# cvg/EMAP

Measured on AMD Instinct MI355X. Metric: ray-samples/sec (UDF MLP + composite), higher is better.
Workload: dtype f16x3 (split-fp16 MFMA, 3 passes, fp32 accumulate)

## Files before the change

### emap_amd/csrc/emap_common.h

```cpp
#pragma once
#include <hip/hip_runtime.h>
#include <stdint.h>
#include <stdio.h>
#include "../../include/emap_hip.h"


namespace emap {
constexpr float F16X3_WS = 8192.0f;
constexpr float F16_LO_SCALE = 2048.0f;

void set_error(const char* fmt, ...);
int check_launch(const char* what);

inline bool attr_needed(uint64_t& mask) {
    int d = 0;
    if (hipGetDevice(&d) != hipSuccess || d < 0 || d > 63) return true;
    if (mask & (1ull << d)) return false;
    mask |= 1ull << d;
    return true;
}
inline int raise_lds_limit(uint64_t& mask, const void* fn, int bytes = 160 * 1024) {
    if (attr_needed(mask) && hipFuncSetAttribute(fn, hipFuncAttributeMaxDynamicSharedMemorySize, bytes) != hipSuccess) {
        set_error("hipFuncSetAttribute(MaxDynamicSharedMemorySize) failed");
        return EMAP_E_LAUNCH;
// ... 63 lines not shown
    const float* rays_d;
    const float* z;
    int32_t n_per_ray;
    int32_t mid;
    const float* sample_dist;
    const float* near;
    const float* far;
    const float* t_rand;
    int32_t coarse;
    int32_t zero_n;
    int32_t* zero_cnt;
};

struct CompositeArgs {
    const float *rays_o, *rays_d, *z, *udf, *grad, *depth_scale, *sample_dist;
    int N, S;
    float inv_s, beta, gamma, car;
    int anneal;
    float flip_sat, near_surface, sparse_scale, background;
    int has_bg;
    const float *var_p, *beta_p, *gamma_p;
    float beta_min;
    EmapCompositeOut out;
    float* partials;
    const float* sched;
};

struct CompositeFuse {
    CompositeArgs c;
    int32_t* ray_cnt;
    int32_t* done_cnt;
};
constexpr int REV_MAX_WG = 768;
constexpr int REV_WG_CAP_4W = REV_MAX_WG * 2 / 3;
constexpr int COMP_LIST_MAX = 8192;
constexpr int COMP_FUSED_MAX_S = 256;
inline long long comp_list_entries(long long P, int S) {
    const long long tiles = (P + 63) / 64, grid = tiles < REV_WG_CAP_4W ? tiles : REV_WG_CAP_4W;
    return ((tiles + grid - 1) / (grid > 0 ? grid : 1)) * (64 / (S > 0 ? S : 1) + 2);
}
struct StepArgs {
    const float *rays_o, *rays_d;
    const float *z, *udf;
    const float *z_prev, *udf_prev;
    float *z_merged, *udf_merged;
    const float *near, *far, *t_rand;
    float* sample_dist;
    float* z_new;
    float* z_final;
    int N, n, m;
    float inv_s, beta, gamma;
    int32_t* err;
};
int launch_sampler_step(bool coarse, bool tail, const StepArgs& a, hipStream_t st, bool plain = false);

struct IsLaunch {
    const float *rays_o, *rays_d, *near, *far, *t_rand;
    float* sample_dist;
    const float* udf_coarse;
    float* z_final;
    int32_t N, Sc, m, steps;
};
constexpr int IS_NOT_FUSED = 1;
int launch_importance(const NetLayout& L, const void* packed, int prec, const IsLaunch& q, hipStream_t st, int32_t* err_flags);
int set_fused_sampling(int on);
int fused_sampling_mode();
int launch_mlp(const NetLayout& L, const void* packed, int prec, const PointSource& src, int64_t P,
               float* udf, float* grad3, hipStream_t st, int32_t* err_flags = nullptr, void* scratch = nullptr,
               const CompositeFuse* fuse = nullptr);
int launch_null_direction(const float* g, int64_t n, int k, float* dir, hipStream_t st);
int launch_lattice_points(int N, int64_t first, int64_t count, float* xyz, hipStream_t st);
size_t compact_workspace_bytes(int64_t n);
int launch_compact_append(const float* df, const float* xyz, int64_t n, int64_t first_index, float thr, int inclusive, float* out_xyz,
                          float* out_df, int64_t* out_idx, int64_t capacity, int64_t* state, void* workspace, hipStream_t st);
int launch_jitter_points(const float* x, const float* noise, int64_t n, int k, float delta, float* out, hipStream_t st);
int launch_shift_points(const float* x, const float* df, const float* normal, int64_t n, float* out, hipStream_t st);

constexpr int VJP_PT = 32;
#ifndef EMAP_VJP_CHUNK_TILES
#define EMAP_VJP_CHUNK_TILES 16384
#endif
constexpr int VJP_CHUNK_TILES = EMAP_VJP_CHUNK_TILES;
constexpr __host__ __device__ int vjp_slab_planes(bool split_f16, bool sweep_mx) { return split_f16 && !sweep_mx ? 6 : 4; }
__device__ __forceinline__ float vjp_scale_from(const uint32_t* absmax) {
    const float mu = __builtin_bit_cast(float, absmax[0]), mg = __builtin_bit_cast(float, absmax[1]);
    const float m = fmaxf(mg, mu * (1.0f / 64.0f));
    if (!(m > 1e-30f) || !(m < 1e30f)) return 1.0f;
    int e;
    (void)frexpf(m, &e);
    return ldexpf(1.0f, -e);
}
constexpr int WGRAD_MAX_JOBS = 2 * EMAP_MAX_LIN;
struct VjpLayout {
    int32_t a_rt[EMAP_MAX_LIN + 1], a_off[EMAP_MAX_LIN + 1];
    int32_t z_rt[EMAP_MAX_LIN], z_off[EMAP_MAX_LIN];
    int32_t s_off[EMAP_MAX_LIN];
    int32_t a_tile_kb, z_tile_kb, s_slab_kb;
    long long lo_a_delta, lo_z_delta;
};
void build_vjp_layout(const NetLayout& L, VjpLayout* V);
struct WgradJob {
    int32_t layer, part;
    int32_t z_off, z_rt;
    int32_t a_off, a_ct;
    int32_t first_wg, n_slices;
    int32_t part_off;
    int32_t bias_off;
};
struct WgradPlan {
    WgradJob jobs[WGRAD_MAX_JOBS];
    int n_jobs, total_wg;
    int job_h[EMAP_MAX_LIN], job_pe[EMAP_MAX_LIN];
    size_t partial_floats;
};
struct VjpSweep {
    PointSource src;
    int64_t P;
    int tile0, n_tiles;
    const float *d_udf, *d_grad;
    const VjpLayout* V;
    char *stash_a, *stash_z, *stash_s;
    int grid;
    const uint32_t* absmax;
    float* ldot;
};

bool mlp_uses_rev(const NetLayout& L, int prec, int64_t P);
int set_grad_mode(int mode);
extern int g_prof_clk_device;
long long* prof_clk_here();
extern long long* g_prof_clk;
constexpr int REV_SG_BYTES_PER_NC = 3072;
inline size_t rev_scratch_bytes(const NetLayout& L) {
    return L.has_rev ? (size_t)REV_WG_CAP_4W * ((size_t)(L.n_lin - 1) * (size_t)(L.H / 32) * (2 * REV_SG_BYTES_PER_NC) + 8192) : 0;
}

int launch_sample_pdf(const float* bins, const float* weights, int N, int n, int m, float* samples, int64_t* inds, int32_t* err,
                      hipStream_t st, const float* u = nullptr);
int launch_upsample(const float* rays_o, const float* rays_d, const float* z, const float* udf, int N, int n, int m, const float* sample_dist,
                    float inv_s, float beta, float gamma, float* z_new, int64_t* inds, int32_t* err, hipStream_t st);
int launch_upsample_plain(const float* z, const float* udf, int N, int n, int m, const float* sample_dist, float beta, float gamma, float* z_new,
                          int64_t* inds, int32_t* err, hipStream_t st);
int launch_merge(const float* z, const float* z_new, const float* udf, const float* udf_new, int N, int n, int m, float* z_out, float* udf_out,
                 int64_t* perm, hipStream_t st);
int launch_coarse(const float* near, const float* far, const float* t_rand, int N, int n_samples, float* z, float* sample_dist, hipStream_t st);
int fill_composite_args(const float* rays_o, const float* rays_d, const float* z, const float* udf, const float* grad3, const float* depth_scale,
                        int N, int S, const float* sample_dist, const EmapRenderParams& p, const EmapCompositeOut* out, float* partials,
                        CompositeArgs* a, const float* sched = nullptr);
int launch_composite(const float* rays_o, const float* rays_d, const float* z, const float* udf, const float* grad3, const float* depth_scale,
                     int N, int S, const float* sample_dist, const EmapRenderParams& p, const EmapCompositeOut* out, float* partials,
                     int32_t* err, hipStream_t st, const float* sched = nullptr);
int launch_composite_reduce(const CompositeArgs& a, int32_t* err, hipStream_t st);
int launch_composite_bwd(const float* rays_o, const float* rays_d, const float* z, const float* udf, const float* grad3, const float* depth_scale,
                         int N, int S, const float* sample_dist, const EmapRenderParams* p, const EmapCompositeGrads* gr, float* d_udf,
                         float* d_grad3, float* partials, uint32_t* absmax, hipStream_t st, const float* sched = nullptr);
int launch_embed(const float* x, int64_t P, int L, float* pe, hipStream_t st);
void linspace_host(float start, float end, int steps, float* out);
int launch_sample_rays(const EmapRayDataset* ds, int img_idx, int batch, int importance, uint64_t seed, uint64_t offset, uint64_t* counter,
                       const int64_t* pixels_in, const EmapRayBatch* out, hipStream_t st);
int check_train_images(const int32_t* images, int n_train, int n_images);
int launch_sample_rays_train(const EmapRayDataset* ds, const int32_t* train_images, int n_train, int32_t* perm, int64_t* epoch_tag, int batch,
                             int importance, uint64_t seed, uint64_t* counter, const int64_t* pixels_in, const EmapRayBatch* out, hipStream_t st);
int gen_rays_count(const EmapRayDataset* ds, int resolution_level, int64_t* n, int* h, int* w);
int launch_gen_rays_at(const EmapRayDataset* ds, int img_idx, int resolution_level, int64_t first, int64_t count, float* rays_o, float* rays_d,
                       float* depth_scale, hipStream_t st);
int launch_train_stats(const float* edge, const float* true_edge, const float* scalars, int N, float d_scale, float* d_edge, float* stats,
// ... 32 lines not shown
```

### emap_amd/csrc/udf_mlp_vjp.inc

```
#pragma once

__device__ __forceinline__ void asm_gload4(uint32_t& dst, int voff, const char* sbase) {
    asm volatile("s_nop 4\n\tglobal_load_dword %0, %1, %2" : "=v"(dst) : "v"(voff), "s"(sbase) : "memory");
}
template <int N>
__device__ __forceinline__ void asm_wait_unit(u32x4& a, u32x4& b, u32x4& c, u32x4& d, u32x2& e, u32x2& f, u32x2& g, u32x2& h, uint32_t& i) {
    asm volatile("s_waitcnt vmcnt(%c9)" : "+v"(a), "+v"(b), "+v"(c), "+v"(d), "+v"(e), "+v"(f), "+v"(g), "+v"(h), "+v"(i) : "i"(N) : "memory");
}


struct VjpArgs {
    MlpArgs m;
    const float* d_udf;
    const float* d_grad;
    char* stash_a;
    char* stash_z;
    char* stash_s;
    const uint32_t* absmax;
    float* ldot;
    VjpLayout V;
    int32_t tile0;
    const char* swm;
    int32_t swm_unit[EMAP_MAX_LIN], swm_t_unit[EMAP_MAX_LIN];
};

template <int H, int MODE, int NW, bool SMX_ = false>
__global__ __launch_bounds__(NW * 64, NW == 8 ? 1 : 2) void udf_mlp_vjp_kernel(const VjpArgs va) {
    using T = typename Prec<MODE>::T;
    using V8 = typename Prec<MODE>::V;
    const MlpArgs& a = va.m;
    constexpr int NPART = Prec<MODE>::NPART;
    constexpr bool SCALED = (NPART == 2);
    constexpr float LO_SCALE = (MODE == EMAP_PREC_F16X3) ? F16_LO_SCALE : 1.0f;
    constexpr int NCT = 4;
    constexpr int NKS = H / 32;
    constexpr int NPAIR = H / 32;
    constexpr int NFR = 2 * NPART;
    constexpr int PD = 2;
    constexpr int PPW = NPAIR / NW;
    constexpr int KQ = NKS / NW;
    static_assert(PPW == 1 && PPW * NW == NPAIR && KQ * NW == NKS && NW >= 4, "waves per workgroup");
    constexpr bool SMX = SMX_ && MODE == EMAP_PREC_F16X3 && H == 256;
    constexpr int NSLAB = vjp_slab_planes(MODE == EMAP_PREC_F16X3, SMX);
    constexpr bool SLABLO = NSLAB > 4;
    typedef uint32_t u32x8 __attribute__((ext_vector_type(8)));

    extern __shared__ __attribute__((aligned(16))) char smem[];
    constexpr int XB = NKS * NCT * NPART * FRAG_BYTES;
    constexpr int PB = PE_KS * NCT * NPART * FRAG_BYTES;
    constexpr bool PP = (NW == 8);
    char* const xb0 = smem;
    char* const xb1 = smem + (PP ? XB : 0);
    char* pebuf = smem + (PP ? 2 : 1) * XB;
    float* red = reinterpret_cast<float*>(PP ? smem + 2 * XB + PB : smem);
    int cur = 0;

    const int tid = threadIdx.x;
    const int lane = tid & 63;
    const int wave = __builtin_amdgcn_readfirstlane(tid >> 6);
    const int g = lane >> 4;
    const int j = lane & 15;
    const int wvoff = lane * 16;
    const char* wbase = uniform_ptr(a.frags);
    const char* tbase = uniform_ptr(a.tfrags);
    const int n_hidden = a.n_lin - 1;
    const char* xr = xb0 + lane * 16;
    const int xm_lane = g * (NCT * NPART * FRAG_BYTES) + FRAG_BYTES;
    const char* xmr = xb0 + xm_lane;
    const char* per = pebuf + lane * 16;
    const int p0 = wave * PPW;
    V8 sel[2];
#pragma unroll
    for (int h = 0; h < 2; ++h)
#pragma unroll
        for (int e = 0; e < 8; ++e) sel[h][e] = ((j >> 2) == g && e == 4 * h + (j & 3)) ? (T)1.0f : (T)0.0f;
    char* const slab = va.stash_s + (size_t)blockIdx.x * ((size_t)va.V.s_slab_kb * 1024);
    const float Kscale = vjp_scale_from(va.absmax);

    clock_stamp(a.clk, 2);
    V8 hd[PD][NFR];
    auto load_head = [&](const char* wb) __attribute__((always_inline)) {
#pragma unroll
        for (int sp = 0; sp < PD; ++sp)
#pragma unroll
            for (int f = 0; f < NFR; ++f) {
                typedef const V8 __attribute__((address_space(1))) * gptr_t;
                hd[sp][f] = *(gptr_t)(uintptr_t)(wb + (sp * NFR + f) * FRAG_BYTES + wvoff);
            }
    };
    u32x2 hd6r[4];
    uint32_t hasc = 0;
    auto load_head_mx = [&](const char* wbh, const char* wm) __attribute__((always_inline)) {
        typedef const V8 __attribute__((address_space(1))) * gptr_t;
        typedef const u32x2 __attribute__((address_space(1))) * g2_t;
        typedef const uint32_t __attribute__((address_space(1))) * g1_t;
#pragma unroll
        for (int sp = 0; sp < PD; ++sp)
#pragma unroll
            for (int t = 0; t < 2; ++t) hd[sp][t] = *(gptr_t)(uintptr_t)(wbh + (sp * NFR + 2 * t) * FRAG_BYTES + wvoff);
#pragma unroll
        for (int t = 0; t < 2; ++t)
#pragma unroll
            for (int pt = 0; pt < 2; ++pt) {
                hd[t][2 + pt] = *(gptr_t)(uintptr_t)(wm + (2 * t + pt) * 1024 + wvoff);
                hd6r[2 * t + pt] = *(g2_t)(uintptr_t)(wm + 4096 + (2 * t + pt) * 512 + lane * 8);
            }
        hasc = *(g1_t)(uintptr_t)(wm + 6144 + lane * 4);
    };
    auto head_after_fwd = [&](int l) __attribute__((always_inline)) {
        int ln = l + 1;
        while (ln < n_hidden && p0 >= a.layer[ln].n_pairs) ++ln;
        const LayerDesc Ln = a.layer[ln < n_hidden ? ln : a.n_lin - 1];
        if constexpr (SMX) {
            if (ln >= n_hidden) return;
            if (!Ln.pe_ks) {
                load_head_mx(wbase + (size_t)(Ln.frag_off + p0 * Ln.h_ks * NFR) * FRAG_BYTES,
                             va.swm + (size_t)(va.swm_unit[ln] + p0 * (NKS / 4)) * SWM_UNIT_BYTES);
                return;
            }
        }
        const int first = (ln < n_hidden) ? p0 * (Ln.pe_ks + Ln.h_ks) : Ln.pe_ks + KQ * wave;
        load_head(wbase + (size_t)(Ln.frag_off + first * NFR) * FRAG_BYTES);
    };
    auto head_after_bwd = [&](int b, int tile) __attribute__((always_inline)) {
        int bn = b - 1;
        while (bn >= 1 && p0 >= a.layer[bn - 1].n_pairs) --bn;
        if (bn >= 1) {
            if constexpr (SMX) load_head_mx(tbase + (size_t)(a.t_off[bn] + p0 * NKS * NFR) * FRAG_BYTES,
                                            va.swm + (size_t)(va.swm_t_unit[bn] + p0 * (NKS / 4)) * SWM_UNIT_BYTES);
            else load_head(tbase + (size_t)(a.t_off[bn] + p0 * NKS * NFR) * FRAG_BYTES);
        }
        else if (tile + (int)gridDim.x < a.n_tiles) head_after_fwd(-1);
    };
    if ((int)blockIdx.x < a.n_tiles) head_after_fwd(-1);
    for (int i = tid * 16; i < (PP ? 2 : 1) * XB; i += NW * 64 * 16) *reinterpret_cast<f32x4*>(smem + i) = f32x4{0.f, 0.f, 0.f, 0.f};
    __syncthreads();
    for (int tile = blockIdx.x; tile < a.n_tiles; tile += gridDim.x) {
        const long long pbase = ((long long)va.tile0 + tile) * VJP_PT;
        char* const sa = va.stash_a + (size_t)tile * ((size_t)va.V.a_tile_kb * 1024);
        char* const sz = va.stash_z + (size_t)tile * ((size_t)va.V.z_tile_kb * 1024);
        constexpr bool LO_STASH = (NPART == 2) && !SMX;
        const bool stash_lo = LO_STASH && va.V.lo_a_delta != 0;
        auto stash_store = [&](char* level_pair, const V8 (&x)[4], int n_rt) __attribute__((always_inline)) {
            const f32x4 z4 = {0.f, 0.f, 0.f, 0.f};
#pragma unroll
            for (int h = 0; h < 2; ++h) {
                if (h < n_rt) {
                    f32x4 d[4];
#pragma unroll
                    for (int ct = 0; ct < 4; ++ct) d[ct] = mfma16(x[ct], sel[h], z4);
#pragma unroll
                    for (int ks = 0; ks < 2; ++ks) {
                        V8 v;
#pragma unroll
                        for (int e = 0; e < 8; ++e) v[e] = (T)d[2 * ks + (e >> 2)][e & 3];
                        *reinterpret_cast<V8*>(level_pair + (h * 2 + ks) * 1024 + lane * 16) = v;
                    }
                }
            }
        };

        if (wave < NCT) {
            const int ct = wave;
            int gq = g;
            asm volatile("" : "+v"(gq));
            float xs[3], vd[3] = {0.f, 0.f, 0.f};
            long long pp = pbase + 16 * (ct & 1) + j;
            const bool valid = pp < a.P;
            if (!valid) pp = a.P - 1;
            load_point(a.src, pp, a.scale, xs);
            if (ct >= 2 && valid) {
                vd[0] = va.d_grad[3 * pp + 0] * Kscale;
                vd[1] = va.d_grad[3 * pp + 1] * Kscale;
                vd[2] = va.d_grad[3 * pp + 2] * Kscale;
            }
            V8 f[PE_KS][NPART];
#pragma unroll
            for (int q = 0; q < 8; ++q) {
                const PeAngle ang = pe_angle(xs, 8 * gq + q, a.multires);
                float v0, v1;
                if (ct < 2) {
                    pe_pair(ang, xs, a.multires, 0, v0, v1);
                } else {
                    const float vc = (ang.c == 0) ? vd[0] : ((ang.c == 1) ? vd[1] : vd[2]);
                    const bool r0 = ang.a == 3 * a.multires, r1 = ang.a == 3 * a.multires + 1;
                    v0 = ang.is_ang ? ang.f * ang.cs * vc : (r0 ? vd[0] : (r1 ? vd[2] : 0.0f));
                    v1 = ang.is_ang ? -ang.f * ang.sn * vc : (r0 ? vd[1] : 0.0f);
                }
                const T h0 = (T)v0, h1 = (T)v1;
                f[q >> 2][0][2 * (q & 3)] = h0;
                f[q >> 2][0][2 * (q & 3) + 1] = h1;
                if constexpr (NPART == 2) {
                    f[q >> 2][1][2 * (q & 3)] = (T)((v0 - (float)h0) * LO_SCALE);
                    f[q >> 2][1][2 * (q & 3) + 1] = (T)((v1 - (float)h1) * LO_SCALE);
                }
            }
#pragma unroll
            for (int sp = 0; sp < PE_KS; ++sp)
#pragma unroll
                for (int pt = 0; pt < NPART; ++pt)
                    *reinterpret_cast<V8*>(pebuf + ((sp * NCT + ct) * NPART + pt) * FRAG_BYTES + lane * 16) = f[sp][pt];
        }
        __syncthreads();
        if (wave >= NW - PE_KS) {
            const int sp = wave - (NW - PE_KS);
            V8 c4[NCT];
#pragma unroll
            for (int ct = 0; ct < NCT; ++ct) c4[ct] = *reinterpret_cast<const V8*>(per + ((sp * NCT + ct) * NPART + 0) * FRAG_BYTES);
            stash_store(sa + (size_t)va.V.a_off[0] * 1024 + (2 * sp) * 2048, c4, 2);
            if constexpr (LO_STASH) {
                if (stash_lo) {
#pragma unroll
                    for (int ct = 0; ct < NCT; ++ct) c4[ct] = *reinterpret_cast<const V8*>(per + ((sp * NCT + ct) * NPART + (NPART - 1)) * FRAG_BYTES);
                    stash_store(sa + va.V.lo_a_delta + (size_t)va.V.a_off[0] * 1024 + (2 * sp) * 2048, c4, 2);
                }
            }
        }

        f32x4 acc[2][NCT];
        f32x4 accx[SCALED ? 2 : 1][NCT];
        V8 o[NCT][NPART];
        const f32x4 zero4 = {0.f, 0.f, 0.f, 0.f};

        auto zval = [&](int t, int ct, int r) __attribute__((always_inline)) -> float {
            if constexpr (SCALED) return fmaf(accx[t][ct][r], 1.0f / LO_SCALE, acc[t][ct][r]);
            else return acc[t][ct][r];
        };

        auto k_run_p = [&](auto ns_c, auto npe_c, auto init_c, auto pre_c, const char* wb, int xs0, int pes0, const float* bp) __attribute__((always_inline)) {
            constexpr int NS = decltype(ns_c)::value;
            constexpr int NPE = decltype(npe_c)::value;
            constexpr bool INIT = decltype(init_c)::value;
            constexpr bool PRE = decltype(pre_c)::value;
            V8 af[PD + 1][NFR];
            auto load_a = [&](auto s_c) __attribute__((always_inline)) {
                constexpr int s = decltype(s_c)::value;
#pragma unroll
                for (int f = 0; f < NFR; ++f) asm_gload16(af[s % (PD + 1)][f], wvoff, wb + (s * NFR + f) * FRAG_BYTES);
            };
            if constexpr (PRE) {
#pragma unroll
                for (int sp = 0; sp < PD; ++sp)
#pragma unroll
                    for (int f = 0; f < NFR; ++f) af[sp][f] = hd[sp][f];
            } else static_for<PD>([&](auto i_c) __attribute__((always_inline)) { if constexpr (decltype(i_c)::value < NS) load_a(i_c); });
            f32x4 i0 = zero4, i1 = zero4;
            if constexpr (INIT) {
                i0 = *reinterpret_cast<const f32x4*>(bp);
                i1 = *reinterpret_cast<const f32x4*>(bp + 16);
            }
            const char* xq = xr + xs0 * (NCT * NPART * FRAG_BYTES);
            const char* pq = per + pes0 * (NCT * NPART * FRAG_BYTES);
            V8 bh[NCT], bl[NCT];
            static_for<NS>([&](auto s_c) __attribute__((always_inline)) {
                constexpr int s = decltype(s_c)::value;
                constexpr int sa_ = s % (PD + 1);
                if constexpr (s == 0 && INIT) asm volatile("" : "+v"(i0), "+v"(i1));
                if constexpr (s + PD < NS) load_a(std::integral_constant<int, s + PD>{});
                constexpr bool is_pe = s < NPE;
                constexpr int sb = is_pe ? s : s - NPE;
#pragma unroll
                for (int ct = 0; ct < NCT; ++ct) {
                    const char* base = is_pe ? pq : xq;
                    bh[ct] = *reinterpret_cast<const V8*>(base + ((sb * NCT + ct) * NPART + 0) * FRAG_BYTES);
                    bl[ct] = *reinterpret_cast<const V8*>(base + ((sb * NCT + ct) * NPART + (NPART - 1)) * FRAG_BYTES);
                }
                {
                    constexpr int younger = ((s + PD < NS) ? PD : (NS - 1 - s)) * NFR;
#pragma unroll
                    for (int f = 0; f < NFR; f += 2) asm_wait_vm<younger>(af[sa_][f], af[sa_][f + 1]);
                }
                if constexpr (s == 0) {
#pragma unroll
                    for (int c2 = 0; c2 < NCT; ++c2) {
                        acc[0][c2] = (c2 < 2) ? i0 : zero4;
                        acc[1][c2] = (c2 < 2) ? i1 : zero4;
                        if constexpr (SCALED) { accx[0][c2] = zero4; accx[1][c2] = zero4; }
                    }
                }
                if constexpr (NPART == 1) {
#pragma unroll
                    for (int ct = 0; ct < NCT; ++ct) {
                        acc[0][ct] = mfma16(af[sa_][0], bh[ct], acc[0][ct]);
                        acc[1][ct] = mfma16(af[sa_][1], bh[ct], acc[1][ct]);
                    }
                } else {
#pragma unroll
                    for (int ct = 0; ct < NCT; ++ct) {
                        if constexpr (SCALED) { accx[0][ct] = mfma16(af[sa_][0], bl[ct], accx[0][ct]); accx[1][ct] = mfma16(af[sa_][2], bl[ct], accx[1][ct]); }
                        else { acc[0][ct] = mfma16(af[sa_][0], bl[ct], acc[0][ct]); acc[1][ct] = mfma16(af[sa_][2], bl[ct], acc[1][ct]); }
                    }
#pragma unroll
                    for (int ct = 0; ct < NCT; ++ct) {
                        acc[0][ct] = mfma16(af[sa_][0], bh[ct], acc[0][ct]);
                        acc[1][ct] = mfma16(af[sa_][2], bh[ct], acc[1][ct]);
                    }
#pragma unroll
// ... 149 lines not shown
                            const auto s02 = __builtin_amdgcn_permlane32_swap(x0, x2, false, false);
                            const auto s13 = __builtin_amdgcn_permlane32_swap(x1, x3, false, false);
                            const auto w01 = __builtin_amdgcn_permlane16_swap(s02[0], s13[0], false, false);
                            const auto w23 = __builtin_amdgcn_permlane16_swap(s02[1], s13[1], false, false);
                            blk[pt][0 * 4 + d] = w01[0]; blk[pt][1 * 4 + d] = w01[1]; blk[pt][2 * 4 + d] = w23[0]; blk[pt][3 * 4 + d] = w23[1];
                        }
                    auto block_max = [&](const u32x16& v) __attribute__((always_inline)) -> float {
                        uint32_t mb = 0;
#pragma unroll
                        for (int q = 0; q < 16; ++q)
                            asm("v_pk_maximum3_f16 %0, %1, %2, %2 neg_lo:[0,0,1] neg_hi:[0,0,1]" : "=v"(mb) : "v"(mb), "v"(v[q]));
                        const h2 m = __builtin_bit_cast(h2, mb);
                        return fmaxf((float)m[0], (float)m[1]);
                    };
                    const uint32_t sbh = mx6_scale_bits(block_max(blk[0])), sbl = mx6_scale_bits(block_max(blk[1]));
                    const u32x6 qh = __builtin_amdgcn_cvt_scalef32_pk32_fp6_f16(__builtin_bit_cast(f16x32, blk[0]), __builtin_bit_cast(float, sbh));
                    const u32x6 ql = __builtin_amdgcn_cvt_scalef32_pk32_fp6_f16(__builtin_bit_cast(f16x32, blk[1]), __builtin_bit_cast(float, sbl));
                    char* const dst = xbuf + ((p0 * NCT + g) * NPART + 1) * FRAG_BYTES;
                    *reinterpret_cast<u32x4*>(dst + j * 16) = u32x4{qh[0], qh[1], qh[2], qh[3]};
                    *reinterpret_cast<u32x4*>(dst + 256 + j * 16) = u32x4{ql[0], ql[1], ql[2], ql[3]};
                    *reinterpret_cast<u32x2*>(dst + 512 + j * 8) = u32x2{qh[4], qh[5]};
                    *reinterpret_cast<u32x2*>(dst + 640 + j * 8) = u32x2{ql[4], ql[5]};
                    *reinterpret_cast<uint32_t*>(dst + 768 + j * 4) = (sbh >> 23) | ((((sbl >> 23) - 11u) & 0xffu) << 8);
                }
            }
            __syncthreads();
            if constexpr (PP) { cur ^= 1; xr = (cur ? xb1 : xb0) + lane * 16; xmr = (cur ? xb1 : xb0) + xm_lane; }
        };
        using yes_t = std::true_type;
        using no_t = std::false_type;
        u32x4 sgv[4];
        auto load_slab = [&](const char* src) __attribute__((always_inline)) {
            const char* sb = uniform_ptr(src);
            static_for<4>([&](auto c_c) __attribute__((always_inline)) {
                constexpr int c = decltype(c_c)::value;
                asm_gload16_sc1<c * 1024>(sgv[c], wvoff, sb);
            });
        };
        auto wait_slab = [&]() __attribute__((always_inline)) {
            asm volatile("s_waitcnt vmcnt(0)" : "+v"(sgv[0]), "+v"(sgv[1]), "+v"(sgv[2]), "+v"(sgv[3]) : : "memory");
        };

        for (int l = 0; l < n_hidden; ++l) {
            const LayerDesc L = a.layer[l];
            const int kind = (L.h_ks == 0) ? KIND_FIRST : (L.pe_ks ? KIND_SKIP : KIND_NORMAL);
            const int p = p0;
            if (p < L.n_pairs) {
                const float* bp = a.bias + l * H + 32 * p + 4 * g;
                const int ns = L.pe_ks + L.h_ks;
                const char* wb = wbase + (size_t)(L.frag_off + p * ns * NFR) * FRAG_BYTES;
                if constexpr (SMX) {
                    const char* wm = va.swm + (size_t)(va.swm_unit[l] + p * (NKS / 4)) * SWM_UNIT_BYTES;
                    if (kind == KIND_NORMAL) k_run_mx(std::integral_constant<int, 1>{}, std::integral_constant<int, NKS / 4>{}, yes_t{}, 0, wb, wm, bp);
                    else if (kind == KIND_SKIP) {
                        k_run_p(std::integral_constant<int, PE_KS>{}, std::integral_constant<int, PE_KS>{}, yes_t{}, yes_t{}, wb, 0, 0, bp);
                        k_run_mx(std::integral_constant<int, 2>{}, std::integral_constant<int, NKS / 4>{}, no_t{}, 0, wb + (size_t)PE_KS * NFR * FRAG_BYTES, wm, bp);
                    } else k_run_p(std::integral_constant<int, PE_KS>{}, std::integral_constant<int, PE_KS>{}, yes_t{}, yes_t{}, wb, 0, 0, bp);
                } else {
                if (kind == KIND_NORMAL) k_run_p(std::integral_constant<int, NKS>{}, std::integral_constant<int, 0>{}, yes_t{}, yes_t{}, wb, 0, 0, bp);
                else if (kind == KIND_SKIP) k_run_p(std::integral_constant<int, PE_KS + NKS>{}, std::integral_constant<int, PE_KS>{}, yes_t{}, yes_t{}, wb, 0, 0, bp);
                else k_run_p(std::integral_constant<int, PE_KS>{}, std::integral_constant<int, PE_KS>{}, yes_t{}, yes_t{}, wb, 0, 0, bp);
                }
                head_after_fwd(l);
                uint32_t bk[SLABLO ? 24 : 16];
                static_for<8>([&](auto q_c) __attribute__((always_inline)) {
                    constexpr int q = decltype(q_c)::value, t = q >> 2, r = q & 3;
                    float a0, s0, a1, s1;
                    softplus_sig_fast(zval(t, 0, r), a0, s0);
                    softplus_sig_fast(zval(t, 1, r), a1, s1);
                    const float t0 = s0 * zval(t, 2, r), t1 = s1 * zval(t, 3, r);
                    put1(0, 4 * t + r, a0);
                    put1(1, 4 * t + r, a1);
                    typedef T T2 __attribute__((ext_vector_type(2)));
                    const T2 ap2 = {put1(2, 4 * t + r, t0), put1(3, 4 * t + r, t1)};
                    bk[2 * q] = __builtin_bit_cast(uint32_t, ap2);
                    bk[2 * q + 1] = __builtin_bit_cast(uint32_t, __builtin_amdgcn_cvt_pknorm_u16(s0, s1));
                    if constexpr (SLABLO) {
                        const T2 lo2 = {(T)((t0 - (float)ap2[0]) * LO_SCALE), (T)((t1 - (float)ap2[1]) * LO_SCALE)};
                        bk[16 + q] = __builtin_bit_cast(uint32_t, lo2);
                    }
                });
                {
                    const V8 xh[4] = {o[0][0], o[1][0], o[2][0], o[3][0]};
                    stash_store(sa + (size_t)va.V.a_off[l + 1] * 1024 + (2 * p) * 2048, xh, 2);
                }
                if constexpr (LO_STASH) {
                    if (stash_lo) {
                        const V8 xl[4] = {o[0][NPART - 1], o[1][NPART - 1], o[2][NPART - 1], o[3][NPART - 1]};
                        stash_store(sa + va.V.lo_a_delta + (size_t)va.V.a_off[l + 1] * 1024 + (2 * p) * 2048, xl, 2);
                    }
                }
                u32x4* dst = reinterpret_cast<u32x4*>(slab + ((size_t)(l * NPAIR + p) * NSLAB) * 1024 + lane * 16);
#pragma unroll
                for (int c = 0; c < NSLAB; ++c) dst[c * 64] = u32x4{bk[4 * c], bk[4 * c + 1], bk[4 * c + 2], bk[4 * c + 3]};
            }
            publish(L.n_pairs);
        }

        float hpart[NCT];
        {
            const LayerDesc L = a.layer[a.n_lin - 1];
            const char* wb = wbase + (size_t)(L.frag_off + (L.pe_ks + KQ * wave) * NFR) * FRAG_BYTES;
            if constexpr (SMX) {
#pragma unroll
                for (int ct = 0; ct < NCT; ++ct) hpart[ct] = 0.f;
                if (wave < NKS / 4) {
                    k_run_mx(std::integral_constant<int, 0>{}, std::integral_constant<int, 1>{}, no_t{}, wave, wbase + (size_t)L.frag_off * FRAG_BYTES,
                             va.swm + (size_t)va.swm_unit[a.n_lin - 1] * SWM_UNIT_BYTES, nullptr);
#pragma unroll
                    for (int ct = 0; ct < NCT; ++ct) hpart[ct] = zval(0, ct, 0);
                }
            } else {
            k_run_p(std::integral_constant<int, KQ>{}, std::integral_constant<int, 0>{}, no_t{}, yes_t{}, wb, KQ * wave, 0, nullptr);
#pragma unroll
            for (int ct = 0; ct < NCT; ++ct) hpart[ct] = zval(0, ct, 0);
            }
            if (L.pe_ks && wave < PE_KS) {
                const char* wp = wbase + (size_t)(L.frag_off + wave * NFR) * FRAG_BYTES;
                k_run(std::integral_constant<int, 1>{}, std::integral_constant<int, 1>{}, no_t{}, wp, 0, wave, nullptr);
#pragma unroll
                for (int ct = 0; ct < NCT; ++ct) hpart[ct] += zval(0, ct, 0);
            }
            head_after_bwd(a.n_lin - 1, tile);
            if constexpr (!PP) __syncthreads();
            if (g == 0) {
#pragma unroll
                for (int ct = 0; ct < NCT; ++ct) red[(wave * NCT + ct) * 16 + j] = hpart[ct];
            }
        }
        __syncthreads();
        float seed[NCT];
        {
            float hs[NCT];
#pragma unroll
            for (int ct = 0; ct < NCT; ++ct) {
                float v = 0.f;
#pragma unroll
                for (int w = 0; w < NW; ++w) v += red[(w * NCT + ct) * 16 + j];
                hs[ct] = v;
            }
            const float b_last = a.bias[(a.n_lin - 1) * H];
            const float inv_scale = 1.0f / a.scale;
            bool bad = false;
#pragma unroll
            for (int c = 0; c < 2; ++c) {
                const long long pp = pbase + 16 * c + j;
                const float h = hs[c] + b_last, hp = hs[c + 2];
                float u1, u2;
                if (a.udf_type == EMAP_UDF_ABS) { u1 = (h > 0.f) ? 1.f : ((h < 0.f) ? -1.f : 0.f); u2 = 0.f; }
                else if (a.udf_type == EMAP_UDF_SQUARE) { u1 = 2.f * h; u2 = 2.f; }
                else { u1 = 1.f; u2 = 0.f; }
                const bool valid = pp < a.P;
                const float du = valid ? va.d_udf[pp] * Kscale : 0.f;
                seed[c] = valid ? fmaf(du * inv_scale, u1, u2 * hp) : 0.f;
                seed[c + 2] = valid ? u1 : 0.f;
                bad |= valid && !(fabsf(h) + fabsf(hp) <= 3.0e38f);
            }
            if (wave == 0 && g == 0) flag_nonfinite(a.err, bad);
            if (wave == 0 && g == 0) {
                float d = seed[0] * hs[0] + seed[1] * hs[1] + seed[2] * hs[2] + seed[3] * hs[3];
#pragma unroll
                for (int off = 8; off > 0; off >>= 1) d += __shfl_xor(d, off);
                if (j == 0) va.ldot[va.tile0 + tile] = d;
            }
        }
        if (wave == 0) {
            V8 xs[4];
#pragma unroll
            for (int ct = 0; ct < NCT; ++ct) {
                const T hi = (T)seed[ct];
#pragma unroll
                for (int e = 0; e < 8; ++e) xs[ct][e] = (T)0.0f;
                xs[ct][0] = (g == 0) ? hi : (T)0.0f;
                xs[ct][1] = (g == 0) ? (T)(seed[ct] - (float)hi) : (T)0.0f;
            }
            stash_store(sz + (size_t)va.V.z_off[a.n_lin - 1] * 1024, xs, 1);
            if constexpr (LO_STASH) {
                if (stash_lo) {
#pragma unroll
                    for (int ct = 0; ct < NCT; ++ct)
#pragma unroll
                        for (int e = 0; e < 8; ++e) xs[ct][e] = (T)0.0f;
                    stash_store(sz + va.V.lo_z_delta + (size_t)va.V.z_off[a.n_lin - 1] * 1024, xs, 1);
                }
            }
        }

        for (int b = a.n_lin - 1; b >= 1; --b) {
            const int lz = b - 1;
            const int p = p0;
            if (p < a.layer[lz].n_pairs) {
                load_slab(slab + ((size_t)(lz * NPAIR + p) * NSLAB) * 1024);
                if (b == a.n_lin - 1) {
                    const f32x4 w0 = *reinterpret_cast<const f32x4*>(a.wlast + 32 * p + 4 * g);
                    const f32x4 w1 = *reinterpret_cast<const f32x4*>(a.wlast + 32 * p + 16 + 4 * g);
#pragma unroll
                    for (int ct = 0; ct < NCT; ++ct) {
                        acc[0][ct] = w0 * seed[ct];
                        acc[1][ct] = w1 * seed[ct];
                        if constexpr (SCALED) { accx[0][ct] = zero4; accx[1][ct] = zero4; }
                    }
                } else {
                    const char* wb = tbase + (size_t)(a.t_off[b] + p * NKS * NFR) * FRAG_BYTES;
                    if constexpr (SMX) k_run_mx(std::integral_constant<int, 0>{}, std::integral_constant<int, NKS / 4>{}, yes_t{}, 0, wb,
                                                va.swm + (size_t)(va.swm_t_unit[b] + p * (NKS / 4)) * SWM_UNIT_BYTES, nullptr);
                    else k_run_p(std::integral_constant<int, NKS>{}, std::integral_constant<int, 0>{}, no_t{}, yes_t{}, wb, 0, 0, nullptr);
                }
                wait_slab();
                u32x4 aplo[2];
                if constexpr (SLABLO) {
                    const char* lp = uniform_ptr(slab + ((size_t)(lz * NPAIR + p) * NSLAB + 4) * 1024);
                    asm_gload16_sc1<0>(aplo[0], wvoff, lp);
                    asm_gload16_sc1<1024>(aplo[1], wvoff, lp);
                    asm volatile("s_waitcnt vmcnt(0)" : "+v"(aplo[0]), "+v"(aplo[1]) : : "memory");
                }
                if (b != a.n_lin - 1) head_after_bwd(b, tile);
                static_for<8>([&](auto q_c) __attribute__((always_inline)) {
                    constexpr int q = decltype(q_c)::value, t = q >> 2, r = q & 3;
                    typedef T T2 __attribute__((ext_vector_type(2)));
                    const uint32_t apk = sgv[q >> 1][2 * (q & 1)], spk = sgv[q >> 1][2 * (q & 1) + 1];
                    const T2 ap2 = __builtin_bit_cast(T2, apk);
                    float ap0 = (float)ap2[0], ap1 = (float)ap2[1];
                    if constexpr (SLABLO) {
                        const uint32_t lok = aplo[q >> 2][q & 3];
                        const T2 lo2 = __builtin_bit_cast(T2, lok);
                        ap0 = fmaf((float)lo2[0], 1.0f / LO_SCALE, ap0);
                        ap1 = fmaf((float)lo2[1], 1.0f / LO_SCALE, ap1);
                    }
                    const float s0 = (float)(spk & 0xffffu) * (1.0f / 65535.0f);
                    const float s1 = (float)(spk >> 16) * (1.0f / 65535.0f);
                    const float av0 = zval(t, 0, r), av1 = zval(t, 1, r), at0 = zval(t, 2, r), at1 = zval(t, 3, r);
                    const float zb0 = fmaf(100.0f * (1.0f - s0) * ap0, at0, s0 * av0);
                    const float zb1 = fmaf(100.0f * (1.0f - s1) * ap1, at1, s1 * av1);
                    put1(0, 4 * t + r, zb0);
                    put1(1, 4 * t + r, zb1);
                    put1(2, 4 * t + r, s0 * at0);
                    put1(3, 4 * t + r, s1 * at1);
                });
                {
                    const V8 xh[4] = {o[0][0], o[1][0], o[2][0], o[3][0]};
                    stash_store(sz + (size_t)va.V.z_off[lz] * 1024 + (2 * p) * 2048, xh, 2);
                }
                if constexpr (LO_STASH) {
                    if (stash_lo) {
                        const V8 xl[4] = {o[0][NPART - 1], o[1][NPART - 1], o[2][NPART - 1], o[3][NPART - 1]};
                        stash_store(sz + va.V.lo_z_delta + (size_t)va.V.z_off[lz] * 1024 + (2 * p) * 2048, xl, 2);
                    }
                }
            }
            if (b > 1) publish(a.layer[lz].n_pairs);
        }
        __syncthreads();
    }
    clock_stamp(a.clk, 3);
}

template <int H, int MODE, int NW, bool SMX_ = false>
static int launch_vjp_sweep_t(const NetLayout& L, const void* packed, const VjpSweep& s, hipStream_t st, int32_t* err) {
    constexpr int NPART = Prec<MODE>::NPART;
    VjpArgs va;
    memset(&va, 0, sizeof(va));
    va.m = fill_mlp_args(L, packed, L.frag_off_bytes, L.t_frag_off_bytes, s.src, s.P, err);
    va.m.n_tiles = s.n_tiles; va.tile0 = s.tile0;
    va.m.clk = prof_clk_here();
    va.d_udf = s.d_udf; va.d_grad = s.d_grad; va.stash_a = s.stash_a; va.stash_z = s.stash_z; va.stash_s = s.stash_s; va.absmax = s.absmax; va.ldot = s.ldot; va.V = *s.V;
    va.swm = static_cast<const char*>(packed) + L.swm_off_bytes;
    for (int l = 0; l < L.n_lin; ++l) { va.swm_unit[l] = L.swm_unit[l]; va.swm_t_unit[l] = L.swm_t_unit[l]; }
    const size_t lds = (NW == 8) ? (size_t)(2 * (H / 32) + PE_KS) * 4 * NPART * FRAG_BYTES + (size_t)NW * 4 * 16 * 4
                                 : (size_t)((H / 32) + PE_KS) * 4 * NPART * FRAG_BYTES;
    auto kern = udf_mlp_vjp_kernel<H, MODE, NW, SMX_>;
    static uint64_t attr_mask = 0;
    const int rc = raise_lds_limit(attr_mask, reinterpret_cast<const void*>(kern));
    if (rc) return rc;
    if (s.n_tiles <= 0) return EMAP_OK;
    hipLaunchKernelGGL(kern, dim3(s.grid < s.n_tiles ? s.grid : s.n_tiles), dim3(NW * 64), lds, st, va);
    return check_launch("udf_mlp_vjp");
}

template <int MODE>
int launch_vjp_sweep_mode(const NetLayout& L, const void* packed, const VjpSweep& s, hipStream_t st, int32_t* err) {
    if constexpr (MODE == EMAP_PREC_F16X3) {
        if (L.H == 256 && L.sweep_mx) return launch_vjp_sweep_t<256, MODE, 8, true>(L, packed, s, st, err);
    }
    if (L.H == 256) return launch_vjp_sweep_t<256, MODE, 8>(L, packed, s, st, err);
    if (L.H == 128) return launch_vjp_sweep_t<128, MODE, 4>(L, packed, s, st, err);
    set_error("no training-backward kernel for d_hidden=%d", L.H);
    return EMAP_E_INVALID;
}
```

### emap_amd/csrc/wgrad.hip

```cpp
#include "emap_common.h"
#include <string.h>

namespace emap {

typedef __bf16 bf16x8 __attribute__((ext_vector_type(8)));
typedef _Float16 f16x8 __attribute__((ext_vector_type(8)));
typedef float f32x4 __attribute__((ext_vector_type(4)));

__device__ __forceinline__ f32x4 mfma16w(const bf16x8& a, const bf16x8& b, const f32x4& c) { return __builtin_amdgcn_mfma_f32_16x16x32_bf16(a, b, c, 0, 0, 0); }
__device__ __forceinline__ f32x4 mfma16w(const f16x8& a, const f16x8& b, const f32x4& c) { return __builtin_amdgcn_mfma_f32_16x16x32_f16(a, b, c, 0, 0, 0); }

__global__ __launch_bounds__(256) void absmax_kernel(const float* du, const float* dg, long long P, uint32_t* out) {
    float mu = 0.f, mg = 0.f;
    for (long long i = (long long)blockIdx.x * 256 + threadIdx.x; i < P; i += (long long)gridDim.x * 256) {
        const float u = fabsf(du[i]);
        const float g = fmaxf(fmaxf(fabsf(dg[3 * i]), fabsf(dg[3 * i + 1])), fabsf(dg[3 * i + 2]));
        mu = (u < 3.0e38f) ? fmaxf(mu, u) : mu;
        mg = (g < 3.0e38f) ? fmaxf(mg, g) : mg;
    }
#pragma unroll
    for (int off = 32; off > 0; off >>= 1) { mu = fmaxf(mu, __shfl_xor(mu, off)); mg = fmaxf(mg, __shfl_xor(mg, off)); }
    if ((threadIdx.x & 63) == 0) {
        atomicMax(out, __builtin_bit_cast(uint32_t, mu));
        atomicMax(out + 1, __builtin_bit_cast(uint32_t, mg));
    }
}

struct WgradArgs {
    const char* stash_a;
    const char* stash_z;
    float* partial;
    int32_t n_tiles, n_jobs, a_tile_kb, z_tile_kb;
    int32_t accumulate;
    float scale;
    int32_t no_bias;
    WgradJob job[WGRAD_MAX_JOBS];
};

template <int CT>
__device__ __forceinline__ void wgrad_store(const WgradArgs& a, const WgradJob& J, int slice, int wave, int lane, f32x4 (&acc)[2][CT], float (&bsum)[2]) {
    float* pb = a.partial + J.part_off + (size_t)slice * 16 * J.a_ct * 256;
#pragma unroll
    for (int i = 0; i < 2; ++i) {
        const int rt = wave + 8 * i;
        if (rt < J.z_rt) {
#pragma unroll
            for (int c = 0; c < CT; ++c) {
                if (c < J.a_ct) {
                    f32x4* dst = reinterpret_cast<f32x4*>(pb + ((size_t)rt * J.a_ct + c) * 256 + lane * 4);
                    *dst = a.accumulate ? (*dst + acc[i][c] * a.scale) : acc[i][c] * a.scale;
                }
            }
        }
    }
    if (J.bias_off >= 0 && !a.no_bias) {
#pragma unroll
        for (int i = 0; i < 2; ++i) {
            float v = bsum[i] * a.scale;
            v += __shfl_xor(v, 16);
            v += __shfl_xor(v, 32);
            const int rt = wave + 8 * i;
            if (rt < J.z_rt && lane < 16) {
                float* dst = a.partial + J.bias_off + (size_t)slice * 256 + rt * 16 + lane;
                *dst = a.accumulate ? (*dst + v) : v;
            }
        }
    }
}

#ifndef EMAP_REDUCE_WAVES
#define EMAP_REDUCE_WAVES 4
#endif
#ifndef EMAP_WGRAD_DEPTH
#define EMAP_WGRAD_DEPTH 3
#endif
constexpr int WGRAD_DEPTH = EMAP_WGRAD_DEPTH;
__device__ __forceinline__ void wg_dma16(unsigned lds_dst, const char* gsrc) {
    unsigned keep;
    asm volatile("s_mov_b32 %0, m0\n\ts_mov_b32 m0, %2\n\ts_nop 0\n\tglobal_load_lds_dwordx4 %1, off\n\ts_mov_b32 m0, %0"
                 : "=&s"(keep) : "v"(gsrc), "s"(lds_dst) : "memory");
}

template <class V8, int NB>
__device__ __forceinline__ void wgrad_lds_run(const WgradArgs& a, const WgradJob& J, int slice, int wave, int lane, char* smem) {
    constexpr int CT = 4 * NB;
    constexpr int NA = (CT + 7) / 8;
    constexpr int NLD = NA + 2;
    constexpr int D = WGRAD_DEPTH, NST = D + 1;
    constexpr int STAGE = (CT + 16) * 1024;
    const int t0 = (int)(((long long)a.n_tiles * slice) / J.n_slices), t1 = (int)(((long long)a.n_tiles * (slice + 1)) / J.n_slices);
    const int nsteps = 2 * (t1 - t0);
    f32x4 acc[2][CT];
#pragma unroll
    for (int i = 0; i < 2; ++i)
#pragma unroll
        for (int c = 0; c < CT; ++c) acc[i][c] = f32x4{0.f, 0.f, 0.f, 0.f};
    float bsum[2] = {0.f, 0.f};
    if (nsteps > 0) {
        const size_t zts = (size_t)a.z_tile_kb * 1024, ats = (size_t)a.a_tile_kb * 1024;
        const char* zsrc = a.stash_z + (size_t)J.z_off * 1024 + lane * 16;
        const char* asrc = a.stash_a + (size_t)J.a_off * 1024 + lane * 16;
        const unsigned lds0 = (unsigned)(size_t)smem;
        int ca[NA], zr[2];
#pragma unroll
        for (int i = 0; i < NA; ++i) ca[i] = 8 * i + ((8 * i + 8 <= CT) ? wave : wave % (CT - 8 * i));
        zr[0] = wave < J.z_rt ? wave : J.z_rt - 1;
        zr[1] = wave + 8 < J.z_rt ? wave + 8 : J.z_rt - 1;
        auto issue = [&](int u) __attribute__((always_inline)) {
            const int uu = u < nsteps ? u : nsteps - 1;
            const int tile = t0 + (uu >> 1), sh = (uu & 1) * 1024;
            const unsigned st = lds0 + (unsigned)(u % NST) * STAGE;
#pragma unroll
            for (int i = 0; i < NA; ++i) {
                const int cs = ca[i] < J.a_ct ? ca[i] : J.a_ct - 1;
                wg_dma16(__builtin_amdgcn_readfirstlane(st + ca[i] * 1024), asrc + (size_t)tile * ats + cs * 2048 + sh);
            }
#pragma unroll
            for (int i = 0; i < 2; ++i)
                wg_dma16(__builtin_amdgcn_readfirstlane(st + (CT + zr[i]) * 1024), zsrc + (size_t)tile * zts + zr[i] * 2048 + sh);
        };
        for (int u = 0; u < D; ++u) issue(u);
        for (int u = 0; u < nsteps; ++u) {
            asm volatile("s_waitcnt vmcnt(%0)" :: "i"(NLD * (D - 1)) : "memory");
            __builtin_amdgcn_s_barrier();
            issue(u + D);
            const char* st = smem + (size_t)(u % NST) * STAGE + lane * 16;
            V8 z[2];
            z[0] = *reinterpret_cast<const V8*>(st + (CT + zr[0]) * 1024);
            z[1] = *reinterpret_cast<const V8*>(st + (CT + zr[1]) * 1024);
            {
                const float m = (u & 1) ? 0.0f : 1.0f;
#pragma unroll
                for (int i = 0; i < 2; ++i)
                    bsum[i] = fmaf(m, (((float)z[i][0] + (float)z[i][1]) + ((float)z[i][2] + (float)z[i][3])) +
                                      (((float)z[i][4] + (float)z[i][5]) + ((float)z[i][6] + (float)z[i][7])), bsum[i]);
            }
#pragma unroll
            for (int c = 0; c < CT; ++c) {
                const V8 af = *reinterpret_cast<const V8*>(st + c * 1024);
                acc[0][c] = mfma16w(z[0], af, acc[0][c]);
                acc[1][c] = mfma16w(z[1], af, acc[1][c]);
            }
        }
        asm volatile("s_waitcnt vmcnt(0)" ::: "memory");
    }
    wgrad_store<CT>(a, J, slice, wave, lane, acc, bsum);
}

#ifdef EMAP_WGRAD_TIMING
static __device__ long long emap_wg_times[1024 * 2];
#endif
template <class V8>
__global__ __launch_bounds__(512, 1) void wgrad_kernel(const WgradArgs a) {
    extern __shared__ __attribute__((aligned(16))) char wg_smem[];
#ifdef EMAP_WGRAD_TIMING
    const long long wg_t0 = __builtin_amdgcn_s_memrealtime();
#endif
    int ji = 0;
    while (ji + 1 < a.n_jobs && (int)blockIdx.x >= a.job[ji + 1].first_wg) ++ji;
    const WgradJob J = a.job[ji];
    const int slice = (int)blockIdx.x - J.first_wg;
    const int lane = threadIdx.x & 63;
    const int wave = __builtin_amdgcn_readfirstlane(threadIdx.x >> 6);
    const int nb = (J.a_ct + 3) >> 2;
    if (nb <= 1) wgrad_lds_run<V8, 1>(a, J, slice, wave, lane, wg_smem);
    else if (nb == 2) wgrad_lds_run<V8, 2>(a, J, slice, wave, lane, wg_smem);
    else if (nb == 3) wgrad_lds_run<V8, 3>(a, J, slice, wave, lane, wg_smem);
    else wgrad_lds_run<V8, 4>(a, J, slice, wave, lane, wg_smem);
#ifdef EMAP_WGRAD_TIMING
    if (threadIdx.x == 0 && blockIdx.x < 1024) { emap_wg_times[2 * blockIdx.x] = ji; emap_wg_times[2 * blockIdx.x + 1] = __builtin_amdgcn_s_memrealtime() - wg_t0; }
#endif
}

struct ReduceArgs {
    const float* partial;
    const uint32_t* absmax;
    const float* ldot;
    int32_t n_tiles;
    float grad_scale;
    int32_t accumulate;
    int32_t weight_norm;
    int32_t n_lin, H, d0, multires, skip_l;
    int32_t row_off[EMAP_MAX_LIN + 1];
    int32_t out_dim[EMAP_MAX_LIN], in_prev[EMAP_MAX_LIN], has_pe[EMAP_MAX_LIN];
    int32_t job_h[EMAP_MAX_LIN], job_pe[EMAP_MAX_LIN];
    WgradJob job[WGRAD_MAX_JOBS];
    const float* g[EMAP_MAX_LIN];
    const float* v[EMAP_MAX_LIN];
    float* dg[EMAP_MAX_LIN];
    float* dv[EMAP_MAX_LIN];
    float* db[EMAP_MAX_LIN];
};

__device__ __forceinline__ float wave_sum_f(float v) {
#pragma unroll
    for (int off = 32; off > 0; off >>= 1) v += __shfl_xor(v, off);
    return v;
}

constexpr int RED_WAVES = EMAP_REDUCE_WAVES;
static_assert(RED_WAVES >= 2 && RED_WAVES <= 16, "EMAP_REDUCE_WAVES: the cross-wave sum needs 2..16 waves (part[RED_WAVES - 1] in LDS)");
__global__ __launch_bounds__(RED_WAVES * 64) void wgrad_reduce_kernel(const ReduceArgs a) {
    __shared__ f32x4 part[RED_WAVES - 1][6][64];
    const int grp = blockIdx.x;
    const int wv = threadIdx.x >> 6;
    const int lane = threadIdx.x & 63;
    if (grp >= a.row_off[a.n_lin]) return;
    int l = 0;
    while (grp >= a.row_off[l + 1]) ++l;
    const int o0 = 4 * (grp - a.row_off[l]);
    const int out_dim = a.out_dim[l];
    const int in_prev = a.in_prev[l];
    const int n_in = in_prev + (a.has_pe[l] ? a.d0 : 0);
    const float inv_k = a.grad_scale / vjp_scale_from(a.absmax);
    const float mult = (l == a.skip_l) ? 0.70710678118654752440f : 1.0f;
    const int rt = o0 >> 4, mq = (o0 & 15) >> 2;
    const bool last = (l == a.n_lin - 1);
    constexpr int MAXC = 6;
    float dw[4][MAXC], vv[4][MAXC];
    float dot[4] = {0.f, 0.f, 0.f, 0.f}, nrm[4] = {0.f, 0.f, 0.f, 0.f};
    const float* src[MAXC];
    size_t str[MAXC];
// ... 237 lines not shown
```

Baseline: 123.9 million.

## Stash raw MFMA fragments and transpose on read with ds_read_tr in wgrad

The forward/VJP stash no longer transposes activation fragments through identity-selector MFMAs before storing. It writes the raw MFMA output fragments in a permuted slot layout, or a half-width layout when only one row tile exists. The wgrad kernel now loads pieces via the new layout and uses ds_read_tr16_b64 LDS transpose reads to rebuild operand fragments. This removes the extra MFMAs and repacking in the stash path, at the cost of more complex LDS addressing and transposed reads in the weight-gradient loop.

Measured after the change: 123.7 million. No clear change (-0.2%).

```diff
diff --git a/emap_amd/csrc/emap_common.h b/emap_amd/csrc/emap_common.h
--- a/emap_amd/csrc/emap_common.h
+++ b/emap_amd/csrc/emap_common.h
@@ -169,6 +169,19 @@
 #endif
 constexpr int VJP_CHUNK_TILES = EMAP_VJP_CHUNK_TILES;
 constexpr __host__ __device__ int vjp_slab_planes(bool split_f16, bool sweep_mx) { return split_f16 && !sweep_mx ? 6 : 4; }
+constexpr int STASH_PAIR_BYTES = 4096;
+constexpr __host__ __device__ int stash_phi(int g, int e) { return 16 * (e >> 2) + 4 * g + (e & 3); }
+constexpr __host__ __device__ int stash_slot(int g, int j) { return 4 * j + g; }
+constexpr __host__ __device__ int stash_lane_bytes(bool half) { return half ? 8 : 16; }
+constexpr __host__ __device__ int stash_frag_bytes(bool half) { return 64 * stash_lane_bytes(half); }
+constexpr __host__ __device__ int stash_store_off(int lane, bool half) { return stash_slot(lane >> 4, lane & 15) * stash_lane_bytes(half); }
+constexpr __host__ __device__ int stash_frag_off(int ct, bool half) { return ct * stash_frag_bytes(half); }
+constexpr __host__ __device__ int stash_kstep_piece_off(int f, int ks, bool half) {
+    return half ? ks * 1024 : (f >> 1) * STASH_PAIR_BYTES + stash_frag_off(2 * ks + (f & 1), false);
+}
+constexpr __host__ __device__ int stash_tr_off(int lane, int h, int c, bool half) {
+    return c * stash_frag_bytes(half) + stash_store_off(16 * (lane & 3) + 4 * (lane >> 4) + ((lane & 15) >> 2), half) + (half ? 0 : 8 * h);
+}
 __device__ __forceinline__ float vjp_scale_from(const uint32_t* absmax) {
     const float mu = __builtin_bit_cast(float, absmax[0]), mg = __builtin_bit_cast(float, absmax[1]);
     const float m = fmaxf(mg, mu * (1.0f / 64.0f));
diff --git a/emap_amd/csrc/udf_mlp_vjp.inc b/emap_amd/csrc/udf_mlp_vjp.inc
--- a/emap_amd/csrc/udf_mlp_vjp.inc
+++ b/emap_amd/csrc/udf_mlp_vjp.inc
@@ -69,11 +69,7 @@
     const char* xmr = xb0 + xm_lane;
     const char* per = pebuf + lane * 16;
     const int p0 = wave * PPW;
-    V8 sel[2];
-#pragma unroll
-    for (int h = 0; h < 2; ++h)
-#pragma unroll
-        for (int e = 0; e < 8; ++e) sel[h][e] = ((j >> 2) == g && e == 4 * h + (j & 3)) ? (T)1.0f : (T)0.0f;
+    const int soff = stash_store_off(lane, false);
     char* const slab = va.stash_s + (size_t)blockIdx.x * ((size_t)va.V.s_slab_kb * 1024);
     const float Kscale = vjp_scale_from(va.absmax);
 
@@ -142,21 +138,13 @@
         constexpr bool LO_STASH = (NPART == 2) && !SMX;
         const bool stash_lo = LO_STASH && va.V.lo_a_delta != 0;
         auto stash_store = [&](char* level_pair, const V8 (&x)[4], int n_rt) __attribute__((always_inline)) {
-            const f32x4 z4 = {0.f, 0.f, 0.f, 0.f};
-#pragma unroll
-            for (int h = 0; h < 2; ++h) {
-                if (h < n_rt) {
-                    f32x4 d[4];
-#pragma unroll
-                    for (int ct = 0; ct < 4; ++ct) d[ct] = mfma16(x[ct], sel[h], z4);
-#pragma unroll
-                    for (int ks = 0; ks < 2; ++ks) {
-                        V8 v;
-#pragma unroll
-                        for (int e = 0; e < 8; ++e) v[e] = (T)d[2 * ks + (e >> 2)][e & 3];
-                        *reinterpret_cast<V8*>(level_pair + (h * 2 + ks) * 1024 + lane * 16) = v;
-                    }
-                }
+            if (n_rt == 2) {
+#pragma unroll
+                for (int ct = 0; ct < 4; ++ct) *reinterpret_cast<V8*>(level_pair + stash_frag_off(ct, false) + soff) = x[ct];
+            } else {
+#pragma unroll
+                for (int ct = 0; ct < 4; ++ct)
+                    *reinterpret_cast<u32x2*>(level_pair + stash_frag_off(ct, true) + stash_store_off(lane, true)) = __builtin_shufflevector(__builtin_bit_cast(u32x4, x[ct]), __builtin_bit_cast(u32x4, x[ct]), 0, 1);
             }
         };
 
@@ -207,12 +195,12 @@
             V8 c4[NCT];
 #pragma unroll
             for (int ct = 0; ct < NCT; ++ct) c4[ct] = *reinterpret_cast<const V8*>(per + ((sp * NCT + ct) * NPART + 0) * FRAG_BYTES);
-            stash_store(sa + (size_t)va.V.a_off[0] * 1024 + (2 * sp) * 2048, c4, 2);
+            stash_store(sa + (size_t)va.V.a_off[0] * 1024 + sp * STASH_PAIR_BYTES, c4, 2);
             if constexpr (LO_STASH) {
                 if (stash_lo) {
 #pragma unroll
                     for (int ct = 0; ct < NCT; ++ct) c4[ct] = *reinterpret_cast<const V8*>(per + ((sp * NCT + ct) * NPART + (NPART - 1)) * FRAG_BYTES);
-                    stash_store(sa + va.V.lo_a_delta + (size_t)va.V.a_off[0] * 1024 + (2 * sp) * 2048, c4, 2);
+                    stash_store(sa + va.V.lo_a_delta + (size_t)va.V.a_off[0] * 1024 + sp * STASH_PAIR_BYTES, c4, 2);
                 }
             }
         }
@@ -528,12 +516,12 @@
                 });
                 {
                     const V8 xh[4] = {o[0][0], o[1][0], o[2][0], o[3][0]};
-                    stash_store(sa + (size_t)va.V.a_off[l + 1] * 1024 + (2 * p) * 2048, xh, 2);
+                    stash_store(sa + (size_t)va.V.a_off[l + 1] * 1024 + p * STASH_PAIR_BYTES, xh, 2);
                 }
                 if constexpr (LO_STASH) {
                     if (stash_lo) {
                         const V8 xl[4] = {o[0][NPART - 1], o[1][NPART - 1], o[2][NPART - 1], o[3][NPART - 1]};
-                        stash_store(sa + va.V.lo_a_delta + (size_t)va.V.a_off[l + 1] * 1024 + (2 * p) * 2048, xl, 2);
+                        stash_store(sa + va.V.lo_a_delta + (size_t)va.V.a_off[l + 1] * 1024 + p * STASH_PAIR_BYTES, xl, 2);
                     }
                 }
                 u32x4* dst = reinterpret_cast<u32x4*>(slab + ((size_t)(l * NPAIR + p) * NSLAB) * 1024 + lane * 16);
@@ -685,12 +673,12 @@
                 });
                 {
                     const V8 xh[4] = {o[0][0], o[1][0], o[2][0], o[3][0]};
-                    stash_store(sz + (size_t)va.V.z_off[lz] * 1024 + (2 * p) * 2048, xh, 2);
+                    stash_store(sz + (size_t)va.V.z_off[lz] * 1024 + p * STASH_PAIR_BYTES, xh, 2);
                 }
                 if constexpr (LO_STASH) {
                     if (stash_lo) {
                         const V8 xl[4] = {o[0][NPART - 1], o[1][NPART - 1], o[2][NPART - 1], o[3][NPART - 1]};
-                        stash_store(sz + va.V.lo_z_delta + (size_t)va.V.z_off[lz] * 1024 + (2 * p) * 2048, xl, 2);
+                        stash_store(sz + va.V.lo_z_delta + (size_t)va.V.z_off[lz] * 1024 + p * STASH_PAIR_BYTES, xl, 2);
                     }
                 }
             }
diff --git a/emap_amd/csrc/wgrad.hip b/emap_amd/csrc/wgrad.hip
--- a/emap_amd/csrc/wgrad.hip
+++ b/emap_amd/csrc/wgrad.hip
@@ -101,33 +101,52 @@
         const char* zsrc = a.stash_z + (size_t)J.z_off * 1024 + lane * 16;
         const char* asrc = a.stash_a + (size_t)J.a_off * 1024 + lane * 16;
         const unsigned lds0 = (unsigned)(size_t)smem;
-        int ca[NA], zr[2];
+        const bool zhalf = J.z_rt == 1;
+        const int a_np = (J.a_ct + 1) & ~1, z_np = zhalf ? 1 : J.z_rt;
+        int ca[NA], zr[2], zp[2];
 #pragma unroll
         for (int i = 0; i < NA; ++i) ca[i] = 8 * i + ((8 * i + 8 <= CT) ? wave : wave % (CT - 8 * i));
-        zr[0] = wave < J.z_rt ? wave : J.z_rt - 1;
-        zr[1] = wave + 8 < J.z_rt ? wave + 8 : J.z_rt - 1;
+#pragma unroll
+        for (int i = 0; i < 2; ++i) {
+            zr[i] = wave + 8 * i < J.z_rt ? wave + 8 * i : J.z_rt - 1;
+            zp[i] = wave + 8 * i < z_np ? wave + 8 * i : z_np - 1;
+        }
         auto issue = [&](int u) __attribute__((always_inline)) {
             const int uu = u < nsteps ? u : nsteps - 1;
-            const int tile = t0 + (uu >> 1), sh = (uu & 1) * 1024;
+            const int tile = t0 + (uu >> 1), ks = uu & 1;
             const unsigned st = lds0 + (unsigned)(u % NST) * STAGE;
 #pragma unroll
             for (int i = 0; i < NA; ++i) {
-                const int cs = ca[i] < J.a_ct ? ca[i] : J.a_ct - 1;
-                wg_dma16(__builtin_amdgcn_readfirstlane(st + ca[i] * 1024), asrc + (size_t)tile * ats + cs * 2048 + sh);
+                const int cs = ca[i] < a_np ? ca[i] : a_np - 1;
+                wg_dma16(__builtin_amdgcn_readfirstlane(st + ca[i] * 1024), asrc + (size_t)tile * ats + stash_kstep_piece_off(cs, ks, false));
             }
 #pragma unroll
             for (int i = 0; i < 2; ++i)
-                wg_dma16(__builtin_amdgcn_readfirstlane(st + (CT + zr[i]) * 1024), zsrc + (size_t)tile * zts + zr[i] * 2048 + sh);
+                wg_dma16(__builtin_amdgcn_readfirstlane(st + (CT + zp[i]) * 1024), zsrc + (size_t)tile * zts + stash_kstep_piece_off(zp[i], ks, zhalf));
         };
+        typedef short i16x4 __attribute__((ext_vector_type(4)));
+        typedef i16x4 __attribute__((address_space(3))) * lds4_t;
+        auto read_tr = [&](unsigned piece0, unsigned o0, unsigned o1) __attribute__((always_inline)) -> V8 {
+            const i16x4 lo = __builtin_amdgcn_ds_read_tr16_b64_v4i16((lds4_t)(uintptr_t)(piece0 + o0));
+            const i16x4 hi = __builtin_amdgcn_ds_read_tr16_b64_v4i16((lds4_t)(uintptr_t)(piece0 + o1));
+            return __builtin_bit_cast(V8, __builtin_shufflevector(lo, hi, 0, 1, 2, 3, 4, 5, 6, 7));
+        };
+        unsigned zo[2][2];
+#pragma unroll
+        for (int i = 0; i < 2; ++i)
+#pragma unroll
+            for (int c = 0; c < 2; ++c) zo[i][c] = (unsigned)((CT + (zhalf ? 0 : zr[i] & ~1)) * 1024 + stash_tr_off(lane, zhalf ? 0 : zr[i] & 1, c, zhalf));
+        const unsigned ao[2][2] = {{(unsigned)stash_tr_off(lane, 0, 0, false), (unsigned)stash_tr_off(lane, 0, 1, false)},
+                                   {(unsigned)stash_tr_off(lane, 1, 0, false), (unsigned)stash_tr_off(lane, 1, 1, false)}};
         for (int u = 0; u < D; ++u) issue(u);
         for (int u = 0; u < nsteps; ++u) {
             asm volatile("s_waitcnt vmcnt(%0)" :: "i"(NLD * (D - 1)) : "memory");
             __builtin_amdgcn_s_barrier();
             issue(u + D);
-            const char* st = smem + (size_t)(u % NST) * STAGE + lane * 16;
+            const unsigned st = lds0 + (unsigned)(u % NST) * STAGE;
             V8 z[2];
-            z[0] = *reinterpret_cast<const V8*>(st + (CT + zr[0]) * 1024);
-            z[1] = *reinterpret_cast<const V8*>(st + (CT + zr[1]) * 1024);
+            z[0] = read_tr(st, zo[0][0], zo[0][1]);
+            z[1] = read_tr(st, zo[1][0], zo[1][1]);
             {
                 const float m = (u & 1) ? 0.0f : 1.0f;
 #pragma unroll
@@ -137,7 +156,7 @@
             }
 #pragma unroll
             for (int c = 0; c < CT; ++c) {
-                const V8 af = *reinterpret_cast<const V8*>(st + c * 1024);
+                const V8 af = read_tr(st + (c & ~1) * 1024, ao[c & 1][0], ao[c & 1][1]);
                 acc[0][c] = mfma16w(z[0], af, acc[0][c]);
                 acc[1][c] = mfma16w(z[1], af, acc[1][c]);
             }
```
